# yashingle-ai/Multi-Modal-Misinformation-Detection-with-Explanation-Generation

Hardware: AMD Instinct MI355X
Metric: text+image pairs/sec through full analyze() 5-signal path, batch=256 (higher is better)
Workload: dtype fp16; 1 GPU; Full MisinfoForensics.analyze() 5-signal pipeline incl. Truth-Vault lookup (BASELINE configs[4]), text L=128, caption L=77, 224x224 images; inputs H2D and results D2H inside the timed region (SURVEY.md §8d); global_batch=256, batch_per_gpu=256, seq_len=128, parallelism=replicas x1 (no data-path collective)

## Files before the change

### include/mmf_hip.h

```cpp
#ifndef MMF_HIP_H
#define MMF_HIP_H

#include <stdint.h>

#ifdef __cplusplus
extern "C" {
#endif

#define MMF_OK 0
#define MMF_EINVAL (-22)
#define MMF_ENOMEM (-12)
#define MMF_EIO (-5)
#define MMF_ERANGE (-34)
#define MMF_EUNSUPPORTED (-95)

#define MMF_DTYPE_F32 0
#define MMF_DTYPE_I64 1

typedef struct mmf_handle mmf_handle;

int mmf_create(int device, mmf_handle** out);
void mmf_destroy(mmf_handle* h);
const char* mmf_last_error(void);
const char* mmf_version(void);
// ... 154 lines not shown

int mmf_gemm_f16(const void* A, int lda, const void* W, int ldw, const float* bias, const float* residual,
                  float* c32, void* c16, int ldc, int M, int N, int K, int act, void* stream);

int mmf_gemm_f16_ex(const void* A, int lda, const void* W, int ldw, const float* bias, const void* res16,
                     const float* ascale, int rows_per_batch, void* c16, int ldc, int M, int N, int K, int act,
                     void* stream);

int mmf_gemm_f16_split(const void* A, int lda, const void* W, int ldw, const float* bias, void* c16, int ldc, int M,
                       int N, int K, int act, int split_lo, void* stream);

int mmf_attention_f16(const void* qkv, const int32_t* mask, void* out, int B, int L, int H, int causal,
                       void* stream);

int mmf_dwconv_nchunks(int H, int W, int C, int stride);
int mmf_dwconv_f16(const void* in, const float* w, const float* bias, void* out, float* pool_part, int B, int H, int W,
                   int C, int k, int stride, int flags, void* stream);
int mmf_expand_dw_f16(const void* x, int cin, const void* we, const float* be, const float* w, const float* bias,
                      void* out, float* pool_part, int B, int H, int W, int C, int k, int stride, int ct, void* stream);
int mmf_se_f32(const float* pool_part, int nchunks, float inv_hw, const float* w1, const float* b1, const float* w2t,
               const float* b2, float* scale, int B, int C, int Csq, int precise, void* stream);
int mmf_effnet_stem_f16(const uint8_t* img_u8, const float* x_f32_nchw, const float* w, const float* bias, void* out,
                        int B, void* stream);
int mmf_effnet_stem_dw_f16(const uint8_t* img_u8, const float* x_f32_nchw, const float* ws, const float* bs,
                           const float* wd, const float* bd, void* out, float* pool_part, int B, void* stream);
int mmf_gap_classifier_f16(const void* x, int HW, int C, const float* w, const float* b, float* logits, float* score,
                           int score_stride, int B, void* stream);

int mmf_pw32_variant(int M, int N, int K, int mfma, int32_t* d_nf_nc);
int mmf_pw32_f32(const float* A, const float* W, const float* bias, const float* ascale, int rows_per_image,
// ... 32 lines not shown
int mmf_gather_rows2(const void* a16, const float* a32, const void* a32h, const int32_t* idx, int L, int C, void* o16,
                     float* o32, int B, void* stream);
int mmf_l2norm_f32(float* x, int B, int C, void* stream);
int mmf_split3_f32(const float* x, int ldx, void* out, int rows, int C, int with_lo, void* stream);
int mmf_attention32_f32(const float* qkv, int ld, int koff, int voff, const int32_t* mask, float* out, int ldo,
                        void* out3, int with_lo, int B, int L, int H, void* stream);
int mmf_attention_q1_f16(const float* q, int ldq, const void* qkv, int ld, int koff, int voff, const int32_t* mask,
                         const int32_t* qpos, void* out, int ldo, int B, int L, int H, void* stream);
int mmf_gemm_splitk_factor(int M, int N, int K, int ldc);
int mmf_gemm_f16_splitk(const void* A, int lda, const void* W, int ldw, const float* bias, const float* res32,
                        const void* res16, float* c32, void* c16, int ldc, int M, int N, int K, int act, float* ws,
                        int64_t ws_elems, void* stream);
int mmf_gemm_f16_raw(const void* A, int lda, const void* W, int ldw, const float* bias, const float* res32,
                     const void* res16, int ldr, const float* ascale, int rows_per_batch, float* c32, void* c16,
                     int ldc, int M, int N, int K, int act, int* config_out, void* stream);
int mmf_gemm_ln_tn(int M, int N, int K);
int mmf_gemm_f16_ln_producer(const void* A, int lda, const void* W, int ldw, const float* bias, const void* res16,
                             void* c16, int ldc, void* ln_out, int M, int N, int K, void* stream);
int mmf_gemm_f16_ln_consumer(const void* A, int lda, const void* W, int ldw, const float* bias, const void* ln_in,
                             int P, int tn, const float* ln_u, float eps, void* c16, int ldc, int M, int N, int K,
                             int act, void* stream);
int mmf_gemm_f16_attn(const void* A, int lda, const void* W, int ldw, const float* bias, const int32_t* amask, void* ctx,
                      int ldc, int M, int N, int K, void* stream);
int mmf_gemm_f16_ln_attn(const void* A, int lda, const void* W, int ldw, const float* bias, const void* ln_in, int P,
                         int tn, const float* ln_u, float eps, const int32_t* amask, int L, int causal, void* ctx,
                         int ldc, int M, int N, int K, void* stream);

int mmf_text_heads_f32(const float* x, int row_stride, const float* w1a_t, const float* b1a, const float* w2a,
                       const float* b2a, const float* w1m_t, const float* b1m, const float* w2m, const float* b2m,
                       float* ai_logits, float* mi_logits, float* scores, int score_stride, const int32_t* ovf, int B,
// ... 28 lines not shown
```

### multi-modal-misinformation-detection-with-explanation-generation_amd/csrc/capi.cpp

```cpp
#include <cmath>
#include <cstdarg>
#include <cstdio>
#include <initializer_list>

#include "handle.h"

thread_local std::string g_err;

int fail(int code, const char* fmt, ...) {
  char buf[1024];
  va_list ap;
  va_start(ap, fmt);
  vsnprintf(buf, sizeof(buf), fmt, ap);
  va_end(ap);
  g_err = buf;
  return code;
}

int free_group(mmf_handle* h, int group) {
  if (h->groups[group].empty()) return 0;
  HIPCHK(hipDeviceSynchronize());
  for (void* p : h->groups[group]) HIPCHK(hipFree(p));
  h->groups[group].clear();
  h->group_bytes[group] = 0;
// ... 9 lines not shown
}

namespace {

struct OptName { const char* name; int Options::*field; const char* env; };
const OptName kOptNames[] = {
    {"concurrent", &Options::concurrent, "MMF_CONCURRENT"},   {"fuse_stem", &Options::fuse_stem, "MMF_FUSE_STEM"},
    {"fuse_expand", &Options::fuse_expand, "MMF_FUSE_EXPAND"},
    {"gemm_splitk", &Options::gemm_splitk, "MMF_GEMM_SPLITK"}, {"gemm_config", &Options::gemm_config, "MMF_GEMM_CONFIG"},
    {"gemm_group_m", &Options::gemm_group_m, "MMF_GEMM_GROUPM"},
    {"text_hilo", &Options::text_hilo, "MMF_TEXT_HILO"}, {"text_prec_mask", &Options::text_prec_mask, "MMF_TEXT_PREC_MASK"},
    {"effnet_fp32", &Options::effnet_fp32, "MMF_EFFNET_FP32"},
    {"clip_res16", &Options::clip_res16, "MMF_CLIP_RES16"}, {"lazy_ln", &Options::lazy_ln, "MMF_LAZY_LN"},
    {"pw32_mfma", &Options::pw32_mfma, "MMF_PW32_MFMA"},
    {"effnet_chunks", &Options::effnet_chunks, "MMF_EFFNET_CHUNKS"}, {"dw_cw32", &Options::dw_cw32, "MMF_DW_CW32"},
    {"diag_skip", &Options::diag_skip, "MMF_DIAG_SKIP"}, {"qkv_attn", &Options::qkv_attn, "MMF_QKV_ATTN"},
    {"clip_qkv_attn", &Options::clip_qkv_attn, "MMF_CLIP_QKV_ATTN"},
    {"vault_ref", &Options::vault_ref, "MMF_VAULT_REF"}, {"vault_fused", &Options::vault_fused, "MMF_VAULT_FUSED"},
    {"mt_enqueue", &Options::mt_enqueue, "MMF_MT_ENQUEUE"}, {"last_q1", &Options::last_q1, "MMF_LAST_Q1"},
    {"after_text", &Options::after_text, "MMF_AFTER_TEXT"},
};
}

Options& process_options() {
  static Options o = [] {
    Options d;
    for (const OptName& n : kOptNames) {
      const char* e = getenv(n.env);
      if (e && *e) d.*(n.field) = atoi(e);
    }
// ... 1109 lines not shown
```

### multi-modal-misinformation-detection-with-explanation-generation_amd/csrc/effnet.hip

```cpp
#include <type_traits>

#include "common.h"
#include "kernels.h"

namespace {

template <typename T>
MMF_DEV T* at_bytes(T* base, uint32_t byte_off) {
  return reinterpret_cast<T*>(reinterpret_cast<char*>(const_cast<typename std::remove_const<T>::type*>(base)) + byte_off);
}

#ifdef MMF_EFF_STAMP
constexpr int kStampBlocks = 16384, kStampSlots = 32;
__device__ unsigned long long* g_eff_stamp;
MMF_DEV unsigned long long est_time() {
  unsigned long long t;
  __builtin_amdgcn_sched_barrier(0);
  asm volatile("s_memtime %0\n\ts_waitcnt lgkmcnt(0)" : "=s"(t) : : "memory");
  __builtin_amdgcn_sched_barrier(0);
  return t;
}
#define EST_BEGIN(REGION)                                                                                   \
  unsigned long long* est_ = nullptr;                                                                        \
  int est_n_ = 2;                                                                                            \
// ... 301 lines not shown
  } else {
    for (int i = tid; i < K * K * CW; i += 256) {
      const int t = i / CW, c = i - t * CW;
      sw[i] = w[(size_t)(c0 + c) * K * K + t];
    }
  }
  for (int i = tid; i < CW; i += 256) sb[i] = bias[c0 + i];
  __syncthreads();
  EST()

  if constexpr (TT > 0)
    dw_compute_ct<K, S, TT, CWT, R>(tile, sw, sb, red, out, pool_part, bi, c0, oy0, ox0, Ho, Wo, C, blockIdx.x, gridDim.x);
  else dw_compute<K, S>(tile, sw, sb, red, out, pool_part, bi, c0, oy0, ox0, Ho, Wo, C, CW, T, IT);
  EST()
  EST_END()
}

#ifndef MMF_EDW_PF
#define MMF_EDW_PF 1
#endif
#ifndef MMF_EDW_PADSKIP
#define MMF_EDW_PADSKIP 1
#endif
template <int K, int S, int KS, int TT, int R, int TPAD>
#ifndef MMF_EDW_MINB1
#define MMF_EDW_MINB1 4
#endif
__global__ __launch_bounds__(256, KS == 1 ? MMF_EDW_MINB1 : KS == 2 ? 3 : 2) void expand_dw_kernel(const f16_t* __restrict__ x, int Cin,
                                                        const f16_t* __restrict__ we, const float* __restrict__ be,
                                                        const float* __restrict__ w, const float* __restrict__ bias,
// ... 510 lines not shown
  for (int t = cap; t >= 1; --t)
    if (Ho % t == 0) { T = t; break; }
  const int tx = (Wo + T - 1) / T, ty = (Ho + T - 1) / T;
  *T_ = T;
  *CW_ = (C % 48 == 0 && !(narrow && C % 32 == 0)) ? 48 : 32;
  *tiles_x_ = tx;
  *ntiles_ = tx * ty;
}

int dwconv_nchunks(int H, int W, int C, int stride) {
  int T, CW, tx, n;
  dw_geometry(H, W, C, stride, &T, &CW, &tx, &n);
  return n;
}

hipError_t launch_dwconv(const f16_t* in, const float* w, const float* bias, f16_t* out, float* pool_part, int B,
                         int H, int W, int C, int k, int stride, int* nchunks_out, hipStream_t s, int ct) {
  int T, CW, tiles_x, ntiles;
  dw_geometry(H, W, C, stride, &T, &CW, &tiles_x, &ntiles, (ct & 8) != 0);
  if (C % CW) return hipErrorInvalidValue;
  *nchunks_out = ntiles;
  const int IT = (T - 1) * stride + k, PX = 256 / (CW / 8);
  const size_t smem = (size_t)dw_tile_bytes(IT, CW, false) + (size_t)(k * k * CW + CW + PX * CW) * 4;
  const size_t smem_ct = (size_t)dw_tile_bytes(IT, CW, true) + (size_t)(k * k * CW + CW) * 4;
  const dim3 grid(ntiles, C / CW, B), blk(256);
#define MMF_DWCT(KK, SS, TT, CC, RR)                                                                          \
  if (k == KK && stride == SS && T == TT && CW == CC) {                                                        \
    hipLaunchKernelGGL((dwconv_kernel<KK, SS, TT, CC, RR>), grid, blk, smem_ct, s, in, w, bias, out, pool_part, H,   \
                       W, C, CW, T, tiles_x);                                                                 \
    return hipGetLastError();                                                                                 \
  }
  if (ct & 1) {
    MMF_DWCT(3, 1, 16, 32, MMF_R_D16)
    MMF_DWCT(3, 1, 14, 32, MMF_R_D14)
    MMF_DWCT(5, 1, 14, 32, MMF_R_D14)
    MMF_DWCT(5, 1, 7, 32, MMF_R_D7)
// ... 112 lines not shown
```

### multi-modal-misinformation-detection-with-explanation-generation_amd/csrc/effnet_host.cpp

```cpp
#include "handle.h"

EffBlock eff_block(int si, int j) {
  const int* st = kStages[si];
  EffBlock B{};
  B.expand = st[0];
  B.k = st[1];
  B.stride = j == 0 ? st[2] : 1;
  B.cin = j == 0 ? st[3] : st[4];
  B.cout = st[4];
  B.cexp = B.cin * B.expand;
  B.csq = B.cin / 4 > 1 ? B.cin / 4 : 1;
  B.residual = (B.stride == 1 && B.cin == B.cout);
  return B;
}

EffSizes eff_sizes() {
  EffSizes z{(size_t)112 * 112 * 32, 0, 0, 0};
  int H = 112;
  for (int si = 0; si < 7; ++si)
    for (int j = 0; j < kStages[si][5]; ++j) {
      const EffBlock b = eff_block(si, j);
      const int Ho = (H - 1) / b.stride + 1;
      z.exp = std::max(z.exp, (size_t)H * H * b.cexp);
      z.dw = std::max(z.dw, (size_t)Ho * Ho * b.cexp);
// ... 101 lines not shown
      ProfScope ps(h, s, PK_DW, 2.0 * B * Ho * Wo * b.cexp * b.k * b.k + 2.0 * B * H * W * b.cin * b.cexp,
                   (double)B * 2 * ((double)H * W * b.cin * (b.cexp / 48) + (double)Ho * Wo * b.cexp));
      HIPCHK(launch_expand_dw(cur, b.cin, b.e.w, b.e.b, b.wd, b.bd, w.e_dw, w.e_pool, B, H, W, b.cexp, b.k, b.stride,
                              &nch, s));
    } else if (b.expand != 1) {
      GemmArgs g = gemm_args(cur, b.cin, b.e, B * H * W);
      g.act = 3;
      g.c16 = w.e_exp;
      CHK(gemm(h, g, s));
      src = w.e_exp;
    }
    if (!fuse && !(&b == &b0 && fuse_stem)) {
      ProfScope ps(h, s, PK_DW, 2.0 * B * Ho * Wo * b.cexp * b.k * b.k,
                   (double)B * b.cexp * 2 * ((double)H * W + (double)Ho * Wo));
      HIPCHK(launch_dwconv(src, b.wd, b.bd, w.e_dw, w.e_pool, B, H, W, b.cexp, b.k, b.stride, &nch, s,
                            1 | (h->opt.dw_cw32 ? 8 : 0)));
    }
    ProfScope ps(h, s, PK_SE, 4.0 * B * b.cexp * b.csq, (double)B * b.cexp * 4 * (nch + 1));
    HIPCHK(launch_se(w.e_pool, nch, 1.0f / (float)(Ho * Wo), b.w1, b.b1, b.w2, b.b2, w.e_scale, B, b.cexp, b.csq, s));
    GemmArgs g = gemm_args(w.e_dw, b.cexp, b.p, B * Ho * Wo);
    g.ascale = w.e_scale;
    g.rows_per_batch = Ho * Wo;
    if (b.residual) g.res16 = cur;
    g.c16 = nxt;
    CHK(gemm(h, g, s));
    std::swap(cur, nxt);
    H = Ho;
    W = Wo;
  }
  GemmArgs g = gemm_args(cur, 320, h->e_head, B * H * W);
  g.act = 3;
// ... 14 lines not shown
}

bool dw_shape_ok(int B, int H, int W, int C, int k, int stride) {
  if (B <= 0 || B > 65535 || H <= 0 || W <= 0 || C <= 0) return false;
  if ((k != 3 && k != 5) || (stride != 1 && stride != 2)) return false;
  return (double)H * W * C * 2.0 < 2147483648.0;
}

}

extern "C" {

int mmf_dwconv_nchunks(int H, int W, int C, int stride) {
  if (H <= 0 || W <= 0 || C <= 0 || (stride != 1 && stride != 2)) return fail(MMF_EINVAL, "dwconv_nchunks: bad shape");
  return dwconv_nchunks(H, W, C, stride);
}

int mmf_dwconv_f16(const void* in, const float* w, const float* bias, void* out, float* pool_part, int B, int H, int W,
                   int C, int k, int stride, int flags, void* stream) {
  if (!in || !w || !bias || !out || !pool_part) return fail(MMF_EINVAL, "null argument");
  if (!dw_shape_ok(B, H, W, C, k, stride))
    return fail(MMF_EINVAL, "dwconv: unsupported shape (B=%d H=%d W=%d C=%d k=%d stride=%d)", B, H, W, C, k, stride);
  int nch = 0;
  return test_launch_rc(launch_dwconv((const f16_t*)in, w, bias, (f16_t*)out, pool_part, B, H, W, C, k, stride, &nch,
                                      (hipStream_t)stream, flags),
                        "dwconv");
}

int mmf_expand_dw_f16(const void* x, int cin, const void* we, const float* be, const float* w, const float* bias,
                      void* out, float* pool_part, int B, int H, int W, int C, int k, int stride, int ct, void* stream) {
// ... 123 lines not shown
```

### multi-modal-misinformation-detection-with-explanation-generation_amd/csrc/gemm.hip

```cpp
#include <type_traits>

#include "common.h"
#include "kernels.h"

namespace {

constexpr int BK = 64;

template <int BM, int BN, int WGM, int WGN>
struct Cfg {
  static constexpr int TM = BM / WGM, TN = BN / WGN;
  static constexpr int MI = TM / 16, NI = TN / 16;
  static constexpr int XC = BM * 8 / 256;
  static constexpr int WC = BN * 8 / 256;
  static_assert(WGM * WGN == 4, "4 waves");
  static_assert(MI >= 1 && NI >= 1, "tile");
  static_assert(XC >= 1 && WC >= 1, "chunking");
};

MMF_DEV int swz(int row, int kc) { return row * BK + ((kc ^ (row & 7)) << 3); }

template <int BM, int BN, int WGM, int WGN, int PF = 1, bool ASC = false>
__global__ __launch_bounds__(256) void gemm_f16_kernel(GemmArgs g, int tilesN) {
  using C = Cfg<BM, BN, WGM, WGN>;
// ... 687 lines not shown
}

static bool glds_ok(const GemmArgs& a) {
  const size_t lim = (size_t)1 << 31;
  const size_t rows = (size_t)a.M + 256;
  const size_t lim32 = (size_t)1 << 32;
  return (a.K % BK) == 0 && !a.ascale && rows * a.ldc * 4 < lim && rows * (a.ldr > 0 ? a.ldr : 0) * 4 < lim &&
         rows * (size_t)a.lda * 2 < lim32 && ((size_t)a.N + 256) * a.ldw * 2 < lim32;
}

#ifndef MMF_GEMM_DIAG
#define MMF_GEMM_DIAG 0
#endif

static bool config_exists(int c) {
  return c == 0 || c == 1 || c == 2 || c == 3 || c == 5 || c == 9 || c == 10 || c == 11 ||
         (MMF_GEMM_DIAG && (c == 15 || c == 16));
}

static int forced_config(const GemmArgs& a) {
  if (a.force_cfg <= 0) return -1;
  const int c = a.force_cfg - 1;
  if (!config_exists(c)) return -1;
  if ((c == 5 || c >= 10) && !glds_ok(a)) return -1;
  if (c == 9 && !pw_applicable(a)) return -1;
  return c;
}

static int glds_pick(const GemmArgs& a, bool with_128) {
  const long tm = (a.M + 255) / 256;
  const int bns[3] = {256, 192, 128}, cfg[3] = {11, 10, 5};
  const double eff[3] = {1.0, 0.88, 0.80};
  int best = 11;
  double bc = 1e30;
  for (int i = 0; i < (with_128 ? 3 : 2); ++i) {
    const long tiles = tm * ((a.N + bns[i] - 1) / bns[i]);
    const double c = (double)((tiles + 255) / 256) * bns[i] / eff[i];
    if (c < bc) { bc = c; best = cfg[i]; }
  }
  return best;
}

int gemm_config(const GemmArgs& a) {
  if (a.epi == 2 || a.epi == 3 || a.epi == 5) return 10;
  const int f = forced_config(a);
  if (a.epi == 1 || a.epi == 4) return (f == 10 || f == 11) ? f : glds_pick(a, false);
  if (f >= 0) return f;
  if (pw_applicable(a)) return 9;
  if (a.N <= 32) return 0;
  if (a.N <= 64) return 1;
  if (a.M <= 512) return 2;
  if (glds_ok(a) && a.N >= 128) return glds_pick(a, true);
  const long t128 = (long)((a.M + 127) / 128) * ((a.N + 127) / 128);
  return t128 < 384 ? 2 : 3;
}

int gemm_splitk_factor(const GemmArgs& a) {
  if (a.ascale || (a.K % 256) || a.K < 512 || (a.N & 3) || (a.ldc & 3) || (a.ldr & 3)) return 1;
  if (a.no_splitk) return 1;
  return a.K / 256;
}

int gemm_ln_tn(const GemmArgs&) { return 96; }
// ... 9 lines not shown
           a.M % 128 == 0 && a.ldc >= a.N / 3;
  if (a.epi == 5)
    return a.ln_in && a.ln_u && a.bias && a.c16 && !a.c32 && !a.res16 && !a.res32 && a.act == ACT_NONE && a.ln_in_P >= 1 &&
           a.ln_in_P <= kLnPMax && a.ln_in_tn > 0 && (long)a.ln_in_P * a.ln_in_tn >= a.K && a.N % 192 == 0 &&
           a.att_L >= 16 && a.att_L <= 128 && a.M % a.att_L == 0 && a.ldc >= a.N / 3;
  if (a.epi == 4)
    return a.c16 && !a.c32 && !a.res16 && !a.res32 && a.bias && a.act == ACT_GELU && a.N % 8 == 0 &&
           a.ldc >= (a.split_lo ? 3 * a.N : a.N) && (size_t)(a.M + 256) * a.ldc * 2 < ((size_t)1 << 31);
  return false;
}

bool gemm_epi_ok(const GemmArgs& a) { return epi_ok(a); }

const char* gemm_config_name(int c) {
  static const char* names[kGemmConfigs] = {
      "gemm_f16<256,32,4,1>", "gemm_f16<256,64,4,1>", "gemm_f16<64,128,1,4>", "gemm_f16<128,128,2,2>", "(removed)",
      "gemm_glds<256,128,4,2>", "(removed)", "(removed)", "(removed)", "pw_conv", "gemm_glds_pipe2<256,192,4,2>",
      "gemm_glds_pipe2<256,256,2,4>", "(removed)", "(removed)", "(removed)", "gemm_glds_dma_only",
      "gemm_glds_compute_only"};
  return (c >= 0 && c < kGemmConfigs) ? names[c] : "gemm_f16<?>";
}

#ifdef MMF_GEMM_STAMP
extern "C" int mmf_debug_gemm_stamp(void* buf) {
  return (int)hipMemcpyToSymbol(HIP_SYMBOL(g_gemm_stamp), &buf, sizeof(buf));
}
#endif

hipError_t launch_gemm(const GemmArgs& a, hipStream_t s) {
  if (a.M <= 0 || a.N <= 0 || a.K <= 0) return hipSuccess;
  if ((a.K & 7) || (a.N & 3) || (a.lda & 7) || (a.ldw & 7) || (a.ldc & 3) || ((a.res32 || a.res16) && (a.ldr & 3)))
// ... 3 lines not shown
    return gemm_config(a) == 11 ? run_glds_epi<256, 256, 2, 4>(a, s) : run_glds_epi<256, 192, 4, 2>(a, s);
  }
  const int cfg = gemm_config(a);
#if MMF_GEMM_DIAG
  if (cfg == 15) return run_glds<256, 192, 4, 2, true, 1>(a, s);
  if (cfg == 16) return run_glds<256, 192, 4, 2, true, 2>(a, s);
#endif
  switch (cfg) {
    case 0: return run<256, 32, 4, 1>(a, s);
    case 1: return run<256, 64, 4, 1>(a, s);
    case 2: {
      const int S = gemm_splitk_factor(a);
      if (S > 1 && a.ws && (size_t)S * a.M * a.N <= a.ws_elems) return run_splitk<64, 128, 1, 4>(a, S, s);
      return run<64, 128, 1, 4>(a, s);
    }
    case 5: return run_glds<256, 128, 4, 2>(a, s);
    case 9: return launch_pw(a, s);
    case 10: return run_glds<256, 192, 4, 2, true>(a, s);
    case 11: return run_glds<256, 256, 2, 4, true>(a, s);
    default: return run<128, 128, 2, 2>(a, s);
  }
}
```

### multi-modal-misinformation-detection-with-explanation-generation_amd/csrc/handle.h

```cpp
#pragma once
#include <hip/hip_runtime.h>

#include <algorithm>
#include <condition_variable>
#include <cstring>
#include <functional>
#include <map>
#include <memory>
#include <mutex>
#include <string>
#include <thread>
#include <vector>

#include "../../include/mmf_hip.h"
#include "kernels.h"

#pragma GCC visibility push(hidden)

extern thread_local std::string g_err;
int fail(int code, const char* fmt, ...);

#define HIPCHK(expr)                                                                      \
  do {                                                                                    \
    hipError_t e_ = (expr);                                                               \
// ... 82 lines not shown

struct Options {
  int concurrent = 1;
  int fuse_stem = 1;
  int fuse_expand = 1;
  int gemm_splitk = 1;
  int gemm_config = -1;
  int gemm_group_m = 0;
  int text_hilo = -1;
  int text_prec_mask = 255;
  int effnet_fp32 = 0;
  int clip_res16 = 1;
  int lazy_ln = 1;
  int pw32_mfma = 5;
  int dw_cw32 = 1;
  int effnet_chunks = 2;
  int qkv_attn = 1;
  int clip_qkv_attn = 1;
  int mt_enqueue = 64;
  int last_q1 = 1;
  int diag_skip = 0;
  int vault_ref = 0;
  int vault_fused = 2;
  int after_text = 12;
};

Options& process_options();

inline void apply_options(const Options& o, GemmArgs* g) {
  g->force_cfg = o.gemm_config >= 0 ? o.gemm_config + 1 : 0;
  g->no_splitk = o.gemm_splitk ? 0 : 1;
  g->group_m = o.gemm_group_m;
}

enum AllocGroup {
  AG_WS = 0, AG_TEXT, AG_EFF, AG_VIS, AG_CTEXT, AG_FUSION, AG_VAULT, AG_TITLES, AG_SIMS, AG_EFF32, AG_RESIZE, AG_TEXT32,
  AG_TP0, AG_TP1, AG_TP2, AG_TP3,
  AG_COUNT
};

enum Ready {
  RDY_TEXT = 1, RDY_EFFNET = 2, RDY_VISION = 4, RDY_CTEXT = 8, RDY_FUSION = 16, RDY_VAULT = 32,
  RDY_CLIP = RDY_VISION | RDY_CTEXT, RDY_MODELS = RDY_TEXT | RDY_EFFNET | RDY_CLIP | RDY_FUSION
};

struct EnqueuePool {
  struct Slot {
// ... 257 lines not shown
```

### multi-modal-misinformation-detection-with-explanation-generation_amd/csrc/kernels.h

```cpp
#pragma once
#include <hip/hip_runtime.h>
#include <stdint.h>

typedef uint16_t f16_t;

struct GemmArgs {
  const f16_t* A;  int lda;
  const f16_t* W;  int ldw;
  const float* bias;
  const float* res32;
  const f16_t* res16;
  int ldr;
  float* c32;
  f16_t* c16;
  int ldc;
  const float* ascale;
  int rows_per_batch;
  int M, N, K, act;
  int force_cfg;
  int no_splitk;
  int group_m;
  float* ws;
  size_t ws_elems;
  int epi;
  const float2* ln_in;
  int ln_in_P, ln_in_tn;
  const float* ln_u;
  float2* ln_out;
  float ln_eps;
  const int32_t* amask;
  int split_lo;
  int att_L, att_causal;
};
bool gemm_epi_ok(const GemmArgs& a);
int gemm_ln_tn(const GemmArgs& a);
int gemm_splitk_factor(const GemmArgs& a);
hipError_t launch_gemm(const GemmArgs& a, hipStream_t s);
int gemm_config(const GemmArgs& a);
constexpr int kGemmConfigs = 17;
const char* gemm_config_name(int c);
bool pw_applicable(const GemmArgs& a);
hipError_t launch_pw(const GemmArgs& a, hipStream_t s);

hipError_t launch_layernorm(const float* x, int ldx, const float* add, int ldadd, const float* g, const float* b,
                            float eps, float* y32, int ldy32, f16_t* y16, int ldy16, int rows, int C,
                            hipStream_t s);

hipError_t launch_add_ln(const float* x, int ldx, const f16_t* y, int ldy, const float* g, const float* b, float eps,
                         float* s32, float* o32, f16_t* o16, int ldo, int rows, int C, hipStream_t s);
hipError_t launch_add_ln(const f16_t* x, int ldx, const f16_t* y, int ldy, const float* g, const float* b, float eps,
                         f16_t* s16, f16_t* o16, int ldo, int rows, int C, hipStream_t s);

hipError_t launch_attention_q1(const float* q, int ldq, const f16_t* qkv, int ld, int koff, int voff,
                               const int32_t* mask, const int32_t* qpos, f16_t* out, int ldo, int B, int L, int H,
                               hipStream_t s);
hipError_t launch_attention(const f16_t* qkv, int ldqkv, const int32_t* mask, f16_t* out, int ldo, int B,
                            int L, int H, int causal, hipStream_t s);
// ... 138 lines not shown
                                 const float* wd, const float* bd, f16_t* out, float* pool_part, int B,
                                 int* nchunks_out, hipStream_t s);
hipError_t launch_dwconv(const f16_t* in, const float* w, const float* bias, f16_t* out, float* pool_part,
                         int B, int H, int W, int C, int k, int stride, int* nchunks_out, hipStream_t s, int ct = 1);
hipError_t launch_se(const float* pool_part, int nchunks, float inv_hw, const float* w1, const float* b1,
                     const float* w2, const float* b2, float* scale, int B, int C, int Csq, hipStream_t s,
                     bool precise = false);
hipError_t launch_gap_classifier(const f16_t* x, int HW, int C, const float* w, const float* b, float* logits,
                                 float* score, int score_stride, int B, hipStream_t s);
hipError_t launch_gap_pooled(const f16_t* x, int HW, int C, float* pooled, int B, hipStream_t s);
hipError_t launch_fill_strided(float* p, int stride, int B, float v, hipStream_t s);
bool expand_dw_applicable(int cin, int cexp, int k);
hipError_t launch_expand_dw(const f16_t* x, int cin, const f16_t* we, const float* be, const float* w,
                            const float* bias, f16_t* out, float* pool_part, int B, int H, int W, int C, int k,
                            int stride, int* nchunks_out, hipStream_t s, int ct = 1);
int dwconv_nchunks(int H, int W, int C, int stride);
hipError_t launch_jpeg_reconstruct(const uint8_t* packed, const uint32_t* block_off, const int64_t* pk_off,
                                   const uint16_t* qt, const int64_t* coef_blocks, const int32_t* infos,
                                   const int64_t* out_offsets, int B, int max_blocks, int max_pixels, uint8_t* samples,
                                   uint8_t* out, hipStream_t s);

constexpr int kResizeKMax = 96;
struct ResizeJob {
  long long src_off;
  int w, h;
  int ow, oh;
  int cx, cy;
  int filt;
  int need_h, need_v;
  int y0, y1;
// ... 24 lines not shown
```

### multi-modal-misinformation-detection-with-explanation-generation_amd/csrc/pointwise.hip

```cpp
#include "common.h"
#include "kernels.h"

namespace {

constexpr int PW_THREADS = 256;
#ifndef PW_SCALE_PRE
#define PW_SCALE_PRE 1
#endif

template <int KS>
MMF_DEV int pw_swz(int r) {
  return (KS & 3) == 0 ? (r & 15) : ((KS & 1) == 0 ? (r & 7) : ((r & 8) >> 2));
}

template <int KS>
constexpr int pw_rpw() {
  return KS <= 2 ? 4 : (KS <= 4 ? 2 : 1);
}

template <int KS, int CF, int ACT>
__global__ __launch_bounds__(PW_THREADS, 4) void pw_kernel(GemmArgs g, int nrb) {
  constexpr int KP = KS * 32, RPW = pw_rpw<KS>(), BN = CF * 16;
  constexpr int ROWS = 4 * RPW * 16;
  constexpr int SLD = BN + 4;
// ... 141 lines not shown
    hipLaunchKernelGGL((pw_kernel<KS, CF, ACT_SILU>), grid, dim3(PW_THREADS), 0, s, a, nrb);
  else if (a.act == ACT_NONE)
    hipLaunchKernelGGL((pw_kernel<KS, CF, ACT_NONE>), grid, dim3(PW_THREADS), 0, s, a, nrb);
  else
    return hipErrorInvalidValue;
  return hipGetLastError();
}

template <int KS>
hipError_t run_pw_ks(const GemmArgs& a, hipStream_t s) {
  if (a.N <= 32) return run_pw<KS, 2>(a, 1, s);
  if (a.N <= 64) return run_pw<KS, 4>(a, 1, s);
  return run_pw<KS, 8>(a, (a.N + 127) / 128, s);
}

}

bool pw_applicable(const GemmArgs& a) {
  if (a.act != ACT_NONE && a.act != ACT_SILU) return false;
  if (a.c32 || a.res32 || !a.c16) return false;
  if ((a.N & 7) || (a.K & 7) || a.K > 256 || a.M < 2048) return false;
  if (!(a.K <= 128 || a.N <= 256)) return false;
  const size_t lim = (size_t)1 << 31;
  const size_t rows = (size_t)a.M + 256;
  return rows * a.lda * 2 < lim && rows * a.ldc * 2 < lim && rows * (a.res16 ? a.ldr : 0) * 2 < lim;
}

hipError_t launch_pw(const GemmArgs& a, hipStream_t s) {
  switch ((a.K + 31) / 32) {
    case 1: return run_pw_ks<1>(a, s);
// ... 11 lines not shown
```

### multi-modal-misinformation-detection-with-explanation-generation_amd/hip.py

```python
from __future__ import annotations

import ctypes
import os

PKG_DIR = os.path.dirname(os.path.abspath(__file__))
LIB_PATH = os.path.join(PKG_DIR, "libmmf_hip.so")

_P = ctypes.c_void_p
_I = ctypes.c_int
_F = ctypes.c_float
_D = ctypes.c_double
SIGNATURES = {
    "mmf_create": (_I, [_I, ctypes.POINTER(_P)]),
    "mmf_destroy": (None, [_P]),
    "mmf_last_error": (ctypes.c_char_p, []),
    "mmf_version": (ctypes.c_char_p, []),
    "mmf_load_tensor": (_I, [_P, ctypes.c_char_p, _I, _I, ctypes.POINTER(ctypes.c_int64), _P]),
    "mmf_finalize": (_I, [_P, _I]),
    "mmf_ready": (_I, [_P]),
    "mmf_reserve": (_I, [_P, _I, _I, _I]),
    "mmf_text_forward": (_I, [_P, _P, _P, _I, _I, _P, _P, _P, _P]),
    "mmf_text_pooled": (_I, [_P, _P, _P, _I, _I, _P, _P]),
    "mmf_head_train_ws_bytes": (ctypes.c_int64, [_I]),
    "mmf_head_train_epoch": (_I, [_P, _P, _I, _P, _P, _F, _I, _P, _D, _D, _D, _D, _D, _I, _P, _P, _P, _P, _P, _P, _P,
# ... 43 lines not shown
    "mmf_mixed_plan": (_I, [_P, _I, _P, _P]),
    "mmf_analyze_mixed": (_I, [_P, _P, _I, _I, _I, _I, _P, _P, _I, _P, _P, _I, _P, _P, _P, _P, _P, _P, _P, _P, _P, _P,
                               _P]),
    "mmf_profile_begin": (_I, [_P]),
    "mmf_profile_end": (_I, [_P, _I, _P, _P, _P, _P]),
    "mmf_profile_kind_name": (ctypes.c_char_p, [_I]),
    "mmf_set_option": (_I, [_P, ctypes.c_char_p, _I]),
    "mmf_get_option": (_I, [_P, ctypes.c_char_p, ctypes.POINTER(_I)]),
    "mmf_option_name": (ctypes.c_char_p, [_I]),
    "mmf_device_bytes": (ctypes.c_int64, [_P]),
    "mmf_gemm_f16": (_I, [_P, _I, _P, _I, _P, _P, _P, _P, _I, _I, _I, _I, _I, _P]),
    "mmf_gemm_f16_ex": (_I, [_P, _I, _P, _I, _P, _P, _P, _I, _P, _I, _I, _I, _I, _I, _P]),
    "mmf_gemm_f16_split": (_I, [_P, _I, _P, _I, _P, _P, _I, _I, _I, _I, _I, _I, _P]),
    "mmf_attention_f16": (_I, [_P, _P, _P, _I, _I, _I, _I, _P]),
    "mmf_dwconv_nchunks": (_I, [_I, _I, _I, _I]),
    "mmf_dwconv_f16": (_I, [_P, _P, _P, _P, _P, _I, _I, _I, _I, _I, _I, _I, _P]),
    "mmf_expand_dw_f16": (_I, [_P, _I, _P, _P, _P, _P, _P, _P, _I, _I, _I, _I, _I, _I, _I, _P]),
    "mmf_se_f32": (_I, [_P, _I, _F, _P, _P, _P, _P, _P, _I, _I, _I, _I, _P]),
    "mmf_effnet_stem_f16": (_I, [_P, _P, _P, _P, _P, _I, _P]),
    "mmf_effnet_stem_dw_f16": (_I, [_P, _P, _P, _P, _P, _P, _P, _P, _I, _P]),
    "mmf_gap_classifier_f16": (_I, [_P, _I, _I, _P, _P, _P, _P, _I, _I, _P]),
    "mmf_pw32_variant": (_I, [_I, _I, _I, _I, _P]),
    "mmf_pw32_f32": (_I, [_P, _P, _P, _P, _I, _P, _P, _I, _I, _I, _I, _I, _P]),
    "mmf_dw32_f32": (_I, [_P, _P, _P, _P, _I, _I, _I, _I, _I, _I, _P]),
    "mmf_sum32_f32": (_I, [_P, _I, _I, _I, _I, _P, _P]),
    "mmf_gap32_f32": (_I, [_P, _I, _I, _P, _P, _P, _P, _I, _I, _P]),
    "mmf_effnet_stem32_f32": (_I, [_P, _P, _P, _P, _P, _I, _P]),
    "mmf_layernorm_f32": (_I, [_P, _I, _P, _I, _P, _P, _F, _P, _I, _P, _I, _I, _I, _P]),
    "mmf_add_ln_f32": (_I, [_P, _I, _P, _I, _P, _P, _F, _P, _P, _P, _I, _I, _I, _P]),
    "mmf_add_ln_f16": (_I, [_P, _I, _P, _I, _P, _P, _F, _P, _P, _I, _I, _I, _P]),
# ... 92 lines not shown
```

Before: 20480 pairs/s.

## Add specialized 7x7 late-stage EfficientNet depthwise and SE-scaled projection kernels

Adds a dedicated depthwise-conv kernel for 7x7 stride-1 late EfficientNet stages. It processes several images per block with register prefetch of the next chunk, fuses SiLU, and writes pooled partials. It also adds a projection GEMM config (64x64 MFMA tile, double-buffered LDS) that applies the per-image SE scale to A while staging it into LDS, and selects it automatically for 49-row-per-image projections. Both are meant to cut the launch and occupancy inefficiency of the generic tiled kernels on tiny 7x7 spatial maps. They add code paths gated by a new effnet_late option, and the smaller tiles may underuse MFMA throughput.

```diff
diff --git a/include/mmf_hip.h b/include/mmf_hip.h
--- a/include/mmf_hip.h
+++ b/include/mmf_hip.h
@@ -192,6 +192,7 @@
                        void* stream);
 
 int mmf_dwconv_nchunks(int H, int W, int C, int stride);
+int mmf_dwconv_late_applicable(int H, int W, int C, int k, int stride);
 int mmf_dwconv_f16(const void* in, const float* w, const float* bias, void* out, float* pool_part, int B, int H, int W,
                    int C, int k, int stride, int flags, void* stream);
 int mmf_expand_dw_f16(const void* x, int cin, const void* we, const float* be, const float* w, const float* bias,
@@ -254,6 +255,7 @@
 int mmf_gemm_f16_raw(const void* A, int lda, const void* W, int ldw, const float* bias, const float* res32,
                      const void* res16, int ldr, const float* ascale, int rows_per_batch, float* c32, void* c16,
                      int ldc, int M, int N, int K, int act, int* config_out, void* stream);
+int mmf_proj_late_selected(int M, int N, int K, int rows_per_batch);
 int mmf_gemm_ln_tn(int M, int N, int K);
 int mmf_gemm_f16_ln_producer(const void* A, int lda, const void* W, int ldw, const float* bias, const void* res16,
                              void* c16, int ldc, void* ln_out, int M, int N, int K, void* stream);
diff --git a/multi-modal-misinformation-detection-with-explanation-generation_amd/csrc/capi.cpp b/multi-modal-misinformation-detection-with-explanation-generation_amd/csrc/capi.cpp
--- a/multi-modal-misinformation-detection-with-explanation-generation_amd/csrc/capi.cpp
+++ b/multi-modal-misinformation-detection-with-explanation-generation_amd/csrc/capi.cpp
@@ -47,6 +47,7 @@
     {"clip_res16", &Options::clip_res16, "MMF_CLIP_RES16"}, {"lazy_ln", &Options::lazy_ln, "MMF_LAZY_LN"},
     {"pw32_mfma", &Options::pw32_mfma, "MMF_PW32_MFMA"},
     {"effnet_chunks", &Options::effnet_chunks, "MMF_EFFNET_CHUNKS"}, {"dw_cw32", &Options::dw_cw32, "MMF_DW_CW32"},
+    {"effnet_late", &Options::effnet_late, "MMF_EFFNET_LATE"},
     {"diag_skip", &Options::diag_skip, "MMF_DIAG_SKIP"}, {"qkv_attn", &Options::qkv_attn, "MMF_QKV_ATTN"},
     {"clip_qkv_attn", &Options::clip_qkv_attn, "MMF_CLIP_QKV_ATTN"},
     {"vault_ref", &Options::vault_ref, "MMF_VAULT_REF"}, {"vault_fused", &Options::vault_fused, "MMF_VAULT_FUSED"},
diff --git a/multi-modal-misinformation-detection-with-explanation-generation_amd/csrc/effnet.hip b/multi-modal-misinformation-detection-with-explanation-generation_amd/csrc/effnet.hip
--- a/multi-modal-misinformation-detection-with-explanation-generation_amd/csrc/effnet.hip
+++ b/multi-modal-misinformation-detection-with-explanation-generation_amd/csrc/effnet.hip
@@ -339,6 +339,121 @@
   else dw_compute<K, S>(tile, sw, sb, red, out, pool_part, bi, c0, oy0, ox0, Ho, Wo, C, CW, T, IT);
   EST()
   EST_END()
+}
+
+constexpr int DL_IPS = 4;
+template <int K>
+__global__ __launch_bounds__(256, 4) void dwconv_late_kernel(const f16_t* __restrict__ in, const float* __restrict__ w,
+                                                           const float* __restrict__ bias, f16_t* __restrict__ out,
+                                                           float* __restrict__ pool_part, int B, int C) {
+  constexpr int PAD = (K - 1) / 2, E = 7, HW = E * E, CW = 32, IPS = DL_IPS;
+  constexpr int NV = IPS * HW * (CW / 8), NL = (NV + 255) / 256;
+  constexpr int TILE_B = IPS * HW * CW * 2, SW_B = K * K * CW * 4, SB_B = CW * 4, RED_B = IPS * HW * CW * 4;
+  __shared__ __attribute__((aligned(16))) unsigned char dl_smem[TILE_B + SW_B + SB_B + RED_B];
+  f16_t* tile = (f16_t*)dl_smem;
+  float* sw = (float*)(dl_smem + TILE_B);
+  float* sb = sw + K * K * CW;
+  float* red = sb + CW;
+  const int tid = threadIdx.x;
+  const int c0 = blockIdx.y * CW;
+  const uint32_t imgb = (uint32_t)HW * C * 2u;
+  const int chunks = (B + IPS - 1) / IPS;
+  int ch = blockIdx.x;
+  if (ch >= chunks) return;
+
+  uint32_t poff[NL];
+#pragma unroll
+  for (int i = 0; i < NL; ++i) {
+    const int idx = tid + i * 256, s = idx / (HW * 4), rem = idx - s * (HW * 4);
+    poff[i] = idx < NV ? (uint32_t)s * imgb + (uint32_t)((rem >> 2) * C + c0 + (rem & 3) * 8) * 2u : kOOB;
+  }
+  u32x4 pre[NL];
+  auto fetch = [&](int chunk) {
+    const int b0 = chunk * IPS;
+    const rsrc_t ri = make_rsrc(in + (size_t)b0 * HW * C, (uint32_t)min(IPS, B - b0) * imgb);
+#pragma unroll
+    for (int i = 0; i < NL; ++i) pre[i] = __builtin_amdgcn_raw_buffer_load_b128(ri, poff[i], 0, 0);
+  };
+  fetch(ch);
+  {
+    constexpr int NW = (K * K * CW + 255) / 256;
+    float wv[NW];
+#pragma unroll
+    for (int j = 0; j < NW; ++j) {
+      const int i = tid + j * 256, t = i / CW, c = i - t * CW;
+      wv[j] = i < K * K * CW ? w[(size_t)(c0 + c) * K * K + t] : 0.f;
+    }
+    const float bv = tid < CW ? bias[c0 + tid] : 0.f;
+#pragma unroll
+    for (int j = 0; j < NW; ++j)
+      if (tid + j * 256 < K * K * CW) sw[tid + j * 256] = wv[j];
+    if (tid < CW) sb[tid] = bv;
+  }
+
+  const int q4 = tid & 7, rw = tid >> 3;
+  const bool live = rw < IPS * E;
+  const int oy = rw % E, si = live ? rw / E : IPS - 1;
+  for (; ch < chunks; ch += gridDim.x) {
+    const int b0 = ch * IPS;
+#pragma unroll
+    for (int i = 0; i < NL; ++i)
+      if (tid + i * 256 < NV) *reinterpret_cast<u32x4*>(tile + (size_t)(tid + i * 256) * 8) = pre[i];
+    if (ch + (int)gridDim.x < chunks) fetch(ch + (int)gridDim.x);
+    __syncthreads();
+    {
+      float acc[E][4];
+      const float4 bv = *reinterpret_cast<const float4*>(sb + q4 * 4);
+#pragma unroll
+      for (int o = 0; o < E; ++o) { acc[o][0] = bv.x; acc[o][1] = bv.y; acc[o][2] = bv.z; acc[o][3] = bv.w; }
+#pragma unroll 1
+      for (int ky = 0; ky < K; ++ky) {
+        float wk[K][4];
+#pragma unroll
+        for (int kx = 0; kx < K; ++kx) {
+          const float4 w0 = *reinterpret_cast<const float4*>(sw + (ky * K + kx) * CW + q4 * 4);
+          wk[kx][0] = w0.x; wk[kx][1] = w0.y; wk[kx][2] = w0.z; wk[kx][3] = w0.w;
+        }
+        const int iy = oy + ky - PAD;
+        const bool rowin = (unsigned)iy < (unsigned)E;
+        const f16_t* row = tile + (size_t)((si * HW + (rowin ? iy : 0) * E) * CW + q4 * 4);
+#pragma unroll
+        for (int col = 0; col < E + K - 1; ++col) {
+          uint2 v = make_uint2(0u, 0u);
+          if (col >= PAD && col < PAD + E) {
+            v = *reinterpret_cast<const uint2*>(row + (col - PAD) * CW);
+            if (!rowin) v = make_uint2(0u, 0u);
+          }
+          const float f[4] = {lo_h(v.x), hi_h(v.x), lo_h(v.y), hi_h(v.y)};
+#pragma unroll
+          for (int o = 0; o < E; ++o) {
+            const int kx = col - o;
+            if (kx >= 0 && kx < K) {
+#pragma unroll
+              for (int j = 0; j < 4; ++j) acc[o][j] = fmaf(f[j], wk[kx][j], acc[o][j]);
+            }
+          }
+        }
+      }
+      const rsrc_t ro = make_rsrc(out + (size_t)b0 * HW * C, (uint32_t)min(IPS, B - b0) * imgb);
+#pragma unroll
+      for (int o = 0; o < E; ++o) {
+        act4<ACT_SILU, true>(acc[o]);
+        if (live)
+          *reinterpret_cast<float4*>(red + (size_t)((si * HW + oy * E + o) * CW + q4 * 4)) =
+              make_float4(acc[o][0], acc[o][1], acc[o][2], acc[o][3]);
+        buf_store_u2(ro, live ? (uint32_t)si * imgb + (uint32_t)((oy * E + o) * C + c0 + q4 * 4) * 2u : kOOB,
+                     make_uint2(pack2h(acc[o][0], acc[o][1]), pack2h(acc[o][2], acc[o][3])));
+      }
+    }
+    __syncthreads();
+    if (tid < IPS * CW) {
+      const int s = tid >> 5, c = tid & 31;
+      float sum = 0.f;
+#pragma unroll
+      for (int q = 0; q < HW; ++q) sum += red[(s * HW + q) * CW + c];
+      if (b0 + s < B) pool_part[(size_t)(b0 + s) * C + c0 + c] = sum;
+    }
+  }
 }
 
 #ifndef MMF_EDW_PF
@@ -879,12 +994,39 @@
   return n;
 }
 
+bool dwconv_late_applicable(int H, int W, int C, int k, int stride) {
+  return H == 7 && W == 7 && stride == 1 && (k == 3 || k == 5) && C > 0 && C % 32 == 0 && C <= 8192;
+}
+
+template <int K>
+static hipError_t run_dwconv_late(const f16_t* in, const float* w, const float* bias, f16_t* out, float* pool_part,
+                                  int B, int C, hipStream_t s) {
+  static const int slots = [] {
+    int dev = 0, cus = 0, occ = 0;
+    if (hipGetDevice(&dev) != hipSuccess ||
+        hipDeviceGetAttribute(&cus, hipDeviceAttributeMultiprocessorCount, dev) != hipSuccess || cus <= 0)
+      cus = 256;
+    if (hipOccupancyMaxActiveBlocksPerMultiprocessor(&occ, dwconv_late_kernel<K>, 256, 0) != hipSuccess || occ <= 0)
+      occ = 4;
+    return cus * occ;
+  }();
+  const int groups = C / 32, chunks = (B + DL_IPS - 1) / DL_IPS;
+  const int bpg_max = slots / groups > 0 ? slots / groups : 1;
+  const int rounds = (chunks + bpg_max - 1) / bpg_max;
+  const int bpg = (chunks + rounds - 1) / rounds;
+  hipLaunchKernelGGL((dwconv_late_kernel<K>), dim3(bpg, groups), dim3(256), 0, s, in, w, bias, out, pool_part, B, C);
+  return hipGetLastError();
+}
+
 hipError_t launch_dwconv(const f16_t* in, const float* w, const float* bias, f16_t* out, float* pool_part, int B,
                          int H, int W, int C, int k, int stride, int* nchunks_out, hipStream_t s, int ct) {
   int T, CW, tiles_x, ntiles;
   dw_geometry(H, W, C, stride, &T, &CW, &tiles_x, &ntiles, (ct & 8) != 0);
   if (C % CW) return hipErrorInvalidValue;
   *nchunks_out = ntiles;
+  if ((ct & 1) && !(ct & 16) && CW == 32 && dwconv_late_applicable(H, W, C, k, stride))
+    return k == 5 ? run_dwconv_late<5>(in, w, bias, out, pool_part, B, C, s)
+                  : run_dwconv_late<3>(in, w, bias, out, pool_part, B, C, s);
   const int IT = (T - 1) * stride + k, PX = 256 / (CW / 8);
   const size_t smem = (size_t)dw_tile_bytes(IT, CW, false) + (size_t)(k * k * CW + CW + PX * CW) * 4;
   const size_t smem_ct = (size_t)dw_tile_bytes(IT, CW, true) + (size_t)(k * k * CW + CW) * 4;
diff --git a/multi-modal-misinformation-detection-with-explanation-generation_amd/csrc/effnet_host.cpp b/multi-modal-misinformation-detection-with-explanation-generation_amd/csrc/effnet_host.cpp
--- a/multi-modal-misinformation-detection-with-explanation-generation_amd/csrc/effnet_host.cpp
+++ b/multi-modal-misinformation-detection-with-explanation-generation_amd/csrc/effnet_host.cpp
@@ -139,7 +139,7 @@
       ProfScope ps(h, s, PK_DW, 2.0 * B * Ho * Wo * b.cexp * b.k * b.k,
                    (double)B * b.cexp * 2 * ((double)H * W + (double)Ho * Wo));
       HIPCHK(launch_dwconv(src, b.wd, b.bd, w.e_dw, w.e_pool, B, H, W, b.cexp, b.k, b.stride, &nch, s,
-                            1 | (h->opt.dw_cw32 ? 8 : 0)));
+                            1 | (h->opt.dw_cw32 ? 8 : 0) | (h->opt.effnet_late ? 0 : 16)));
     }
     ProfScope ps(h, s, PK_SE, 4.0 * B * b.cexp * b.csq, (double)B * b.cexp * 4 * (nch + 1));
     HIPCHK(launch_se(w.e_pool, nch, 1.0f / (float)(Ho * Wo), b.w1, b.b1, b.w2, b.b2, w.e_scale, B, b.cexp, b.csq, s));
@@ -184,6 +184,10 @@
 int mmf_dwconv_nchunks(int H, int W, int C, int stride) {
   if (H <= 0 || W <= 0 || C <= 0 || (stride != 1 && stride != 2)) return fail(MMF_EINVAL, "dwconv_nchunks: bad shape");
   return dwconv_nchunks(H, W, C, stride);
+}
+
+int mmf_dwconv_late_applicable(int H, int W, int C, int k, int stride) {
+  return dwconv_late_applicable(H, W, C, k, stride) ? 1 : 0;
 }
 
 int mmf_dwconv_f16(const void* in, const float* w, const float* bias, void* out, float* pool_part, int B, int H, int W,
diff --git a/multi-modal-misinformation-detection-with-explanation-generation_amd/csrc/gemm.hip b/multi-modal-misinformation-detection-with-explanation-generation_amd/csrc/gemm.hip
--- a/multi-modal-misinformation-detection-with-explanation-generation_amd/csrc/gemm.hip
+++ b/multi-modal-misinformation-detection-with-explanation-generation_amd/csrc/gemm.hip
@@ -725,7 +725,7 @@
 #endif
 
 static bool config_exists(int c) {
-  return c == 0 || c == 1 || c == 2 || c == 3 || c == 5 || c == 9 || c == 10 || c == 11 ||
+  return c == 0 || c == 1 || c == 2 || c == 3 || c == 4 || c == 5 || c == 9 || c == 10 || c == 11 ||
          (MMF_GEMM_DIAG && (c == 15 || c == 16));
 }
 
@@ -735,6 +735,7 @@
   if (!config_exists(c)) return -1;
   if ((c == 5 || c >= 10) && !glds_ok(a)) return -1;
   if (c == 9 && !pw_applicable(a)) return -1;
+  if (c == 4 && !proj_late_applicable(a)) return -1;
   return c;
 }
 
@@ -758,6 +759,7 @@
   if (a.epi == 1 || a.epi == 4) return (f == 10 || f == 11) ? f : glds_pick(a, false);
   if (f >= 0) return f;
   if (pw_applicable(a)) return 9;
+  if (!a.no_late && proj_late_applicable(a)) return 4;
   if (a.N <= 32) return 0;
   if (a.N <= 64) return 1;
   if (a.M <= 512) return 2;
@@ -797,7 +799,7 @@
 
 const char* gemm_config_name(int c) {
   static const char* names[kGemmConfigs] = {
-      "gemm_f16<256,32,4,1>", "gemm_f16<256,64,4,1>", "gemm_f16<64,128,1,4>", "gemm_f16<128,128,2,2>", "(removed)",
+      "gemm_f16<256,32,4,1>", "gemm_f16<256,64,4,1>", "gemm_f16<64,128,1,4>", "gemm_f16<128,128,2,2>", "proj_late<64,64,2,2>",
       "gemm_glds<256,128,4,2>", "(removed)", "(removed)", "(removed)", "pw_conv", "gemm_glds_pipe2<256,192,4,2>",
       "gemm_glds_pipe2<256,256,2,4>", "(removed)", "(removed)", "(removed)", "gemm_glds_dma_only",
       "gemm_glds_compute_only"};
@@ -831,6 +833,7 @@
       if (S > 1 && a.ws && (size_t)S * a.M * a.N <= a.ws_elems) return run_splitk<64, 128, 1, 4>(a, S, s);
       return run<64, 128, 1, 4>(a, s);
     }
+    case 4: return launch_proj_late(a, s);
     case 5: return run_glds<256, 128, 4, 2>(a, s);
     case 9: return launch_pw(a, s);
     case 10: return run_glds<256, 192, 4, 2, true>(a, s);
diff --git a/multi-modal-misinformation-detection-with-explanation-generation_amd/csrc/handle.h b/multi-modal-misinformation-detection-with-explanation-generation_amd/csrc/handle.h
--- a/multi-modal-misinformation-detection-with-explanation-generation_amd/csrc/handle.h
+++ b/multi-modal-misinformation-detection-with-explanation-generation_amd/csrc/handle.h
@@ -120,6 +120,7 @@
   int lazy_ln = 1;
   int pw32_mfma = 5;
   int dw_cw32 = 1;
+  int effnet_late = 1;
   int effnet_chunks = 2;
   int qkv_attn = 1;
   int clip_qkv_attn = 1;
@@ -137,6 +138,7 @@
   g->force_cfg = o.gemm_config >= 0 ? o.gemm_config + 1 : 0;
   g->no_splitk = o.gemm_splitk ? 0 : 1;
   g->group_m = o.gemm_group_m;
+  g->no_late = o.effnet_late ? 0 : 1;
 }
 
 enum AllocGroup {
diff --git a/multi-modal-misinformation-detection-with-explanation-generation_amd/csrc/kernels.h b/multi-modal-misinformation-detection-with-explanation-generation_amd/csrc/kernels.h
--- a/multi-modal-misinformation-detection-with-explanation-generation_amd/csrc/kernels.h
+++ b/multi-modal-misinformation-detection-with-explanation-generation_amd/csrc/kernels.h
@@ -20,6 +20,7 @@
   int force_cfg;
   int no_splitk;
   int group_m;
+  int no_late;
   float* ws;
   size_t ws_elems;
   int epi;
@@ -41,6 +42,8 @@
 const char* gemm_config_name(int c);
 bool pw_applicable(const GemmArgs& a);
 hipError_t launch_pw(const GemmArgs& a, hipStream_t s);
+bool proj_late_applicable(const GemmArgs& a);
+hipError_t launch_proj_late(const GemmArgs& a, hipStream_t s);
 
 hipError_t launch_layernorm(const float* x, int ldx, const float* add, int ldadd, const float* g, const float* b,
                             float eps, float* y32, int ldy32, f16_t* y16, int ldy16, int rows, int C,
@@ -209,6 +212,7 @@
 hipError_t launch_expand_dw(const f16_t* x, int cin, const f16_t* we, const float* be, const float* w,
                             const float* bias, f16_t* out, float* pool_part, int B, int H, int W, int C, int k,
                             int stride, int* nchunks_out, hipStream_t s, int ct = 1);
+bool dwconv_late_applicable(int H, int W, int C, int k, int stride);
 int dwconv_nchunks(int H, int W, int C, int stride);
 hipError_t launch_jpeg_reconstruct(const uint8_t* packed, const uint32_t* block_off, const int64_t* pk_off,
                                    const uint16_t* qt, const int64_t* coef_blocks, const int32_t* infos,
diff --git a/multi-modal-misinformation-detection-with-explanation-generation_amd/csrc/pointwise.hip b/multi-modal-misinformation-detection-with-explanation-generation_amd/csrc/pointwise.hip
--- a/multi-modal-misinformation-detection-with-explanation-generation_amd/csrc/pointwise.hip
+++ b/multi-modal-misinformation-detection-with-explanation-generation_amd/csrc/pointwise.hip
@@ -179,6 +179,168 @@
   return run_pw<KS, 8>(a, (a.N + 127) / 128, s);
 }
 
+constexpr int PL_BM = 64, PL_BN = 64, PL_BK = 64, PL_KMAX = 1152, PL_RPB = 49, PL_IMGS = 3;
+MMF_DEV int pl_swz(int row, int kc) { return row * PL_BK + ((kc ^ (row & 7)) << 3); }
+
+__global__ __launch_bounds__(256, 3) void proj_late_kernel(GemmArgs g, int tilesN) {
+  constexpr int BM = PL_BM, BN = PL_BN, BK = PL_BK, STAGE = (BM + BN) * BK;
+  __shared__ __attribute__((aligned(16))) unsigned char pl_smem[2 * STAGE * 2 + PL_IMGS * PL_KMAX * 4];
+  f16_t* lds = (f16_t*)pl_smem;
+  float* ssc = (float*)(pl_smem + 2 * STAGE * 2);
+  auto Xs = [&](int buf) { return lds + buf * STAGE; };
+  auto Ws = [&](int buf) { return lds + buf * STAGE + BM * BK; };
+
+  const int nwg = gridDim.x, bid = blockIdx.x;
+  const int xcd = bid & 7, q = nwg >> 3, r = nwg & 7;
+  const int wgid = (xcd < r ? xcd * (q + 1) : r * (q + 1) + (xcd - r) * q) + (bid >> 3);
+  const int tm = wgid / tilesN, tn = wgid - tm * tilesN;
+  const int m0 = tm * BM, n0 = tn * BN;
+  const int tid = threadIdx.x, lane = tid & 63, wave = tid >> 6;
+  const int wm = wave >> 1, wn = wave & 1;
+  const int fr = lane & 15, fg = lane >> 4;
+  const int M = g.M, N = g.N, K = g.K;
+  const int nk = (K + BK - 1) / BK;
+
+  const rsrc_t ra = make_rsrc(g.A, ((uint32_t)(M - 1) * g.lda + K) * 2u);
+  const rsrc_t rw = make_rsrc(g.W, ((uint32_t)(N - 1) * g.ldw + K) * 2u);
+  const rsrc_t rs = make_rsrc(g.ascale, (uint32_t)((M - 1) / PL_RPB + 1) * K * 4u);
+  const rsrc_t rr = make_rsrc(g.res16, g.res16 ? ((uint32_t)(M - 1) * g.ldr + N) * 2u : 0u);
+  const rsrc_t rc = make_rsrc(g.c16, ((uint32_t)(M - 1) * g.ldc + N) * 2u);
+
+  const int img0 = m0 / PL_RPB, kq4 = K >> 2;
+  constexpr int NS = (PL_IMGS * PL_KMAX / 4 + 255) / 256;
+  float4 sv[NS];
+#pragma unroll
+  for (int i = 0; i < NS; ++i) {
+    const int idx = tid + i * 256, li = idx / kq4, kq = idx - li * kq4;
+    sv[i] = buf_load_f4(rs, li < PL_IMGS ? ((uint32_t)(img0 + li) * K + kq * 4) * 4u : kOOB);
+  }
+
+  const int kc = tid & 7;
+  uint32_t aoff[2], woff[2];
+  int sbase[2];
+#pragma unroll
+  for (int i = 0; i < 2; ++i) {
+    const int row = (tid >> 3) + 32 * i;
+    aoff[i] = ((uint32_t)(m0 + row) * g.lda + kc * 8) * 2u;
+    woff[i] = ((uint32_t)(n0 + row) * g.ldw + kc * 8) * 2u;
+    sbase[i] = (min(m0 + row, M - 1) / PL_RPB - img0) * K + kc * 8;
+  }
+  u32x4 xa[2], wa[2], xb[2], wb[2];
+  auto load_to = [&](int kt, u32x4* xd, u32x4* wd) {
+    const bool in = kt * BK + kc * 8 < K;
+#pragma unroll
+    for (int i = 0; i < 2; ++i) {
+      xd[i] = __builtin_amdgcn_raw_buffer_load_b128(ra, in ? aoff[i] + (uint32_t)kt * (BK * 2) : kOOB, 0, 0);
+      wd[i] = __builtin_amdgcn_raw_buffer_load_b128(rw, in ? woff[i] + (uint32_t)kt * (BK * 2) : kOOB, 0, 0);
+    }
+  };
+  auto store_from = [&](int buf, int kt, const u32x4* xs, const u32x4* ws) {
+    const bool in = kt * BK + kc * 8 < K;
+#pragma unroll
+    for (int i = 0; i < 2; ++i) {
+      const int row = (tid >> 3) + 32 * i;
+      u32x4 v = xs[i];
+      if (in) {
+        const float4 s0 = *reinterpret_cast<const float4*>(ssc + sbase[i] + kt * BK);
+        const float4 s1 = *reinterpret_cast<const float4*>(ssc + sbase[i] + kt * BK + 4);
+        v.x = pack2h(lo_h(v.x) * s0.x, hi_h(v.x) * s0.y);
+        v.y = pack2h(lo_h(v.y) * s0.z, hi_h(v.y) * s0.w);
+        v.z = pack2h(lo_h(v.z) * s1.x, hi_h(v.z) * s1.y);
+        v.w = pack2h(lo_h(v.w) * s1.z, hi_h(v.w) * s1.w);
+      }
+      *reinterpret_cast<u32x4*>(Xs(buf) + pl_swz(row, kc)) = v;
+      *reinterpret_cast<u32x4*>(Ws(buf) + pl_swz(row, kc)) = ws[i];
+    }
+  };
+
+  load_to(0, xb, wb);
+  load_to(1, xa, wa);
+#pragma unroll
+  for (int i = 0; i < NS; ++i)
+    if (tid + i * 256 < PL_IMGS * kq4) *reinterpret_cast<float4*>(ssc + (size_t)(tid + i * 256) * 4) = sv[i];
+  __syncthreads();
+  store_from(0, 0, xb, wb);
+  __syncthreads();
+
+  f32x4 acc[2][2];
+#pragma unroll
+  for (int i = 0; i < 2; ++i)
+#pragma unroll
+    for (int j = 0; j < 2; ++j) acc[i][j] = f32x4{0.f, 0.f, 0.f, 0.f};
+  auto compute = [&](int buf) {
+#pragma unroll
+    for (int ks = 0; ks < 2; ++ks) {
+      f16x8 wf[2], xf[2];
+#pragma unroll
+      for (int i = 0; i < 2; ++i)
+        wf[i] = as_f16x8(*reinterpret_cast<const uint4*>(Ws(buf) + pl_swz(wn * 32 + i * 16 + fr, ks * 4 + fg)));
+#pragma unroll
+      for (int j = 0; j < 2; ++j)
+        xf[j] = as_f16x8(*reinterpret_cast<const uint4*>(Xs(buf) + pl_swz(wm * 32 + j * 16 + fr, ks * 4 + fg)));
+#pragma unroll
+      for (int i = 0; i < 2; ++i)
+#pragma unroll
+        for (int j = 0; j < 2; ++j) acc[i][j] = mfma16x16x32(wf[i], xf[j], acc[i][j]);
+    }
+  };
+  for (int kt = 0; kt + 1 < nk; kt += 2) {
+    load_to(kt + 2, xb, wb);
+    compute(0);
+    store_from(1, kt + 1, xa, wa);
+    __syncthreads();
+    load_to(kt + 3, xa, wa);
+    compute(1);
+    store_from(0, kt + 2, xb, wb);
+    __syncthreads();
+  }
+  if (nk & 1) compute(0);
+
+  const int mb = m0 + wm * 32 + fr, nb = n0 + wn * 32 + fg * 4;
+  float4 bv[2];
+  uint2 r16[2][2];
+#pragma unroll
+  for (int i = 0; i < 2; ++i) {
+    bv[i] = g.bias ? *reinterpret_cast<const float4*>(g.bias + nb + i * 16) : make_float4(0.f, 0.f, 0.f, 0.f);
+#pragma unroll
+    for (int j = 0; j < 2; ++j)
+      r16[i][j] = buf_load_u2(rr, ((uint32_t)(mb + j * 16) * g.ldr + nb + i * 16) * 2u);
+  }
+  const bool has_res = g.res16 != nullptr;
+#pragma unroll
+  for (int j = 0; j < 2; ++j)
+#pragma unroll
+    for (int i = 0; i < 2; ++i) {
+      float v[4] = {acc[i][j][0] + bv[i].x, acc[i][j][1] + bv[i].y, acc[i][j][2] + bv[i].z, acc[i][j][3] + bv[i].w};
+      if (has_res) {
+        v[0] += lo_h(r16[i][j].x); v[1] += hi_h(r16[i][j].x); v[2] += lo_h(r16[i][j].y); v[3] += hi_h(r16[i][j].y);
+      }
+      const int m = mb + j * 16;
+      buf_store_u2(rc, m < M ? ((uint32_t)m * g.ldc + nb + i * 16) * 2u : kOOB,
+                   make_uint2(pack2h(v[0], v[1]), pack2h(v[2], v[3])));
+    }
+}
+
+}
+
+bool proj_late_applicable(const GemmArgs& a) {
+  if (!a.ascale || a.rows_per_batch != PL_RPB || a.act != ACT_NONE || a.epi != 0) return false;
+  if (a.c32 || a.res32 || !a.c16) return false;
+  if ((a.N % PL_BN) || a.N > 320 || (a.K & 7) || a.K <= 256 || a.K > PL_KMAX) return false;
+  if ((a.lda & 7) || (a.ldw & 7) || (a.ldc & 3) || (a.res16 && (a.ldr & 3 || a.ldr < a.N)) || a.lda < a.K || a.ldw < a.K ||
+      a.ldc < a.N)
+    return false;
+  const size_t lim = (size_t)1 << 31;
+  const size_t rows = (size_t)a.M + PL_BM;
+  return rows * a.lda * 2 < lim && rows * a.ldc * 2 < lim && rows * (a.res16 ? a.ldr : 0) * 2 < lim &&
+         (size_t)a.N * a.ldw * 2 < lim && (rows / PL_RPB + 1) * a.K * 4 < lim;
+}
+
+hipError_t launch_proj_late(const GemmArgs& a, hipStream_t s) {
+  if (!proj_late_applicable(a)) return hipErrorInvalidValue;
+  const int tilesM = (a.M + PL_BM - 1) / PL_BM, tilesN = a.N / PL_BN;
+  hipLaunchKernelGGL(proj_late_kernel, dim3(tilesM * tilesN), dim3(256), 0, s, a, tilesN);
+  return hipGetLastError();
 }
 
 bool pw_applicable(const GemmArgs& a) {
diff --git a/multi-modal-misinformation-detection-with-explanation-generation_amd/hip.py b/multi-modal-misinformation-detection-with-explanation-generation_amd/hip.py
--- a/multi-modal-misinformation-detection-with-explanation-generation_amd/hip.py
+++ b/multi-modal-misinformation-detection-with-explanation-generation_amd/hip.py
@@ -81,6 +81,8 @@
     "mmf_gemm_f16_split": (_I, [_P, _I, _P, _I, _P, _P, _I, _I, _I, _I, _I, _I, _P]),
     "mmf_attention_f16": (_I, [_P, _P, _P, _I, _I, _I, _I, _P]),
     "mmf_dwconv_nchunks": (_I, [_I, _I, _I, _I]),
+    "mmf_dwconv_late_applicable": (_I, [_I, _I, _I, _I, _I]),
+    "mmf_proj_late_selected": (_I, [_I, _I, _I, _I]),
     "mmf_dwconv_f16": (_I, [_P, _P, _P, _P, _P, _I, _I, _I, _I, _I, _I, _I, _P]),
     "mmf_expand_dw_f16": (_I, [_P, _I, _P, _P, _P, _P, _P, _P, _I, _I, _I, _I, _I, _I, _I, _P]),
     "mmf_se_f32": (_I, [_P, _I, _F, _P, _P, _P, _P, _P, _I, _I, _I, _I, _P]),
```

Measured after the change: 20560 pairs/s, median of 6. About the same (+0.4%).
